# mpetri/ans-large-alphabet

Hardware: AMD Instinct MI355X
Metric: encode+decode Mints/s (uint32), bit-exact vs CPU reference per block (higher is better)
Workload: dtype u32 symbols; ANS state carried as an exact f64 (integers below 2^53) in the encoder, u64 in the decoder; 1 GPU; ANSfold-1 on 268435456 uint32 per GPU, zipf20s1.2, blocks of 16384 ints, restart every 1024; codec=ANSfold-1, ints_per_gpu=268435456, distribution=zipf20s1.2, block_ints=16384, ckpt_interval=1024, seed=1234, multi_gpu=single GPU

## Files before the change

### ans_large_alphabet_amd/csrc/ansx.hip

```cpp
#include "../../include/ansx.h"

#include <hip/hip_runtime.h>
#include <dlfcn.h>
#include <rccl/rccl.h>

#include <algorithm>
#include <array>
#include <cmath>
#include <cstdio>
#include <cstdlib>
#include <cstring>
#include <deque>
#include <map>
#include <set>
#include <string>
#include <vector>

#include "ansx_kernels.h"
#include "ansx_rfold.h"
#include "ansx_model.h"
#include "ansx_fastmodel.h"
#include "ansx_gen.h"
#include "ansx_pa.h"
#include "ansx_intsparse.h"
// ... 22 lines not shown
    hipStream_t stream = nullptr;
    int last_hip = 0;
    bool profile = false;
    std::vector<ProfRec> recs;
    std::map<std::string, std::pair<double, u64>> acc;
    std::vector<std::string> order;
    DevBuf pre_work;
    DevBuf hist, hterm, sortF, sortSym, attS, prevS, attMeta, blk, table, tab32, scratch, misc, mapped, mostfreq,
        stage_in, stage_out, dec_s2s, dec_cum, dec_info, plain, rf_tmp, log2lut, pa_alpha, pa_info, pairs, lg2i, sizes, nearlist, force;
    u32* h_pin = nullptr;
    std::map<u64, u32> ns_hint;
    std::map<u64, u32> rf_hint;
    std::map<std::array<u64, 4>, ansx_container_header> hdr_cache;
    std::deque<std::array<u64, 4>> hdr_order;
    std::map<u32, DevBuf> geo;
    DevBuf geo_big;
    u32 geo_big_cap = 0;
    int last_gather_ranks = 0;
    std::set<u64> wide_hint;
    std::map<u64, u32> t_hint;
    const u32* cur_force = nullptr;
    const u32* cur_src = nullptr;
    bool used_pc = false;
    bool used_fast = false;
    u32 cur_nt = 0;
    u32 cur_rf_slots = 0;
    u32 cur_pa_distinct = 0;
    std::set<u64> int_sparse_hint;
    bool cur_int_sparse = false;
    u32 sp_retries = 0;
    bool sp_full_lds = false;
    ansx_encode_stats last = {};
    struct {
        bool table16_fixup = false;
        bool encode_gtab16 = false;
        bool parse_generic = false;
        bool parse_win = false;
        bool parse_fast = false;
        bool decode_table = false;
        bool no_stream_lds = false;
        int decode_mode = 0;
        u32 parse_stage_words = 0;
        bool model_fused = false;
        bool model_sync = false;
        bool use_pc = false;
        u32 pc_b_pairs = 2;
        u32 test_sp_bits = 0;
        bool fin_one_wave = false;
        bool no_big_geo = false;
        bool no_pc_auto = false;
        bool encode_mode2 = false;
        bool force_pc = false;
        bool no_pc = false;
        int decode_small_ring = 0;
        int decode_pair = 0;
        u32 pair_lds_limit = 0;
        u32 wide_at = 16;
        bool wide_restart = false;
        u32 ns_hint = 0;
        u32 t_hint = 0;
        bool no_fast_model = false;
        double near_band = ANSX_NEAR_BAND;
        bool near_flip = false;
        u32 cand_chains = 0;
        double fast_guard = ANSX_FAST_GUARD;
    } dbg;
};

namespace {

#define HIPCHK(ctx, call)                                                                        \
    do {                                                                                         \
        hipError_t _e = (call);                                                                  \
        if (_e != hipSuccess) {                                                                  \
            (ctx)->last_hip = (int)_e;                                                           \
            return ANSX_ERR_HIP;                                                                 \
        }                                                                                        \
    } while (0)

int ensure(ansx_ctx* c, DevBuf& b, size_t bytes)
{
    if (bytes <= b.cap) return ANSX_OK;
    if (b.p) {
        hipError_t e = hipFree(b.p);
        b.p = nullptr;
        b.cap = 0;
        if (e != hipSuccess) {
            c->last_hip = (int)e;
            return ANSX_ERR_HIP;
        }
    }
    size_t want = bytes + (bytes >> 3) + 4096;
    hipError_t e = hipMalloc(&b.p, want);
    if (e != hipSuccess) {
        c->last_hip = (int)e;
        return ANSX_ERR_HIP;
    }
    b.cap = want;
    return ANSX_OK;
}

void prof_begin(ansx_ctx* c, const char* name, hipStream_t s)
{
    if (!c->profile) return;
    ProfRec r;
    r.name = name;
// ... 153 lines not shown
        LAUNCH(c, "k_rfg_insert", k_rfg_insert, grid, 256, 0, s, d_in, g, slots, keys, counts, bstat);
        if ((size_t)T * 8 > 48 * 1024)
            HIPCHK(c, hipFuncSetAttribute((const void*)k_rfg_select,
                          hipFuncAttributeMaxDynamicSharedMemorySize, (int)((size_t)T * 8)));
        LAUNCH(c, "k_rfg_select", k_rfg_select, g.nblocks, 256, (size_t)T * 8, s, g, slots, (const u32*)keys,
            counts, (const u32*)bstat, mostfreq, blk, gflags);
        LAUNCH(c, "k_rfg_map", k_rfg_map, grid, 256, 0, s, d_in, g, slots, (const u32*)keys, (const u32*)counts,
            (const ansx_blk*)blk, mapped);
        return ANSX_OK;
    }
    if (T <= 4096) {
        const size_t sel_bytes = 8 * (size_t)(T < 512 ? 512 : T);
        if (opt_slots != 0 && opt_slots < ANSX_RF_SLOTS) {
            const size_t lds = 6 * (size_t)opt_slots + sel_bytes;
            HIPCHK(c, hipFuncSetAttribute((const void*)k_rfold_remap_hash2,
                          hipFuncAttributeMaxDynamicSharedMemorySize, (int)lds));
#ifdef ANSX_STAMPS_RF
            { static unsigned long long z[3] = { 0, 0, 0 }; (void)hipMemcpyToSymbol(HIP_SYMBOL(g_stamps), z, 24, 4101 * 8); }
            hipEvent_t e0, e1; (void)hipEventCreate(&e0); (void)hipEventCreate(&e1); (void)hipEventRecord(e0, s);
#endif
            LAUNCH(c, "k_rfold_remap", k_rfold_remap_hash2, g.nblocks, 1024, lds, s, d_in, g, opt_slots, mapped,
                mostfreq, blk, gflags);
#ifdef ANSX_STAMPS_RF
            {
                (void)hipEventRecord(e1, s); (void)hipStreamSynchronize(s);
                float ms = 0; (void)hipEventElapsedTime(&ms, e0, e1);
                unsigned long long z[3]; (void)hipMemcpyFromSymbol(z, HIP_SYMBOL(g_stamps), 24, 4101 * 8);
                fprintf(stderr, "[stamps] k_rfold_remap_hash2: events %.3f ms; workgroup lifetimes: max %llu ticks, mean %.0f ticks, %llu above 40 us\n", ms, z[0], (double)z[1] / g.nblocks, z[2]);
            }
#endif
            return ANSX_OK;
        }
        const size_t lds = 6 * (size_t)ANSX_RF_SLOTS + sel_bytes;
        HIPCHK(c, hipFuncSetAttribute((const void*)k_rfold_remap_hash,
                      hipFuncAttributeMaxDynamicSharedMemorySize, (int)lds));
        LAUNCH(c, "k_rfold_remap", k_rfold_remap_hash, g.nblocks, 1024, lds, s, d_in, g, (u32)ANSX_RF_SLOTS, mapped,
            mostfreq, blk, gflags);
        return ANSX_OK;
    }
    u32 N2 = 2;
    while (N2 < g.block_ints) N2 <<= 1;
    size_t lds = 6 * (size_t)N2 + 8 * (size_t)T + 16;
    if (lds > 48 * 1024)
        HIPCHK(c, hipFuncSetAttribute((const void*)k_rfold_remap,
                      hipFuncAttributeMaxDynamicSharedMemorySize, (int)lds));
    LAUNCH(c, "k_rfold_remap_sort", k_rfold_remap, g.nblocks, 256, lds, s, d_in, g, N2, mapped, mostfreq,
        blk, gflags);
    return ANSX_OK;
}

constexpr int ANSX_RETRY_GENERAL = -1;
constexpr int ANSX_RETRY_WIDE = -2;

template <bool POW2, int S>
static int launch_pc(ansx_ctx* c, const ansx_geo& g, u32 NSP, const u32* src, u32 ns_entries, u32 rowwords, u32 pairs, u32 wgs,
    size_t lds, ansx_blk* blk, u64 scr_stride, u64* ck_state, u32* ck_off, u32* enc_sizes, unsigned long long* enc_gsums, hipStream_t s)
{
    HIPCHK(c, hipFuncSetAttribute((const void*)k_encode_pc<POW2, S>, hipFuncAttributeMaxDynamicSharedMemorySize, (int)lds));
    LAUNCH(c, "k_encode", (k_encode_pc<POW2, S>), wgs, 128 * pairs, lds, s, src, g, NSP, (const u32*)c->tab32.p, ns_entries, rowwords, blk,
        (u8*)c->scratch.p, scr_stride, ck_state, ck_off, enc_sizes, enc_gsums);
    return ANSX_OK;
}
static int launch_f64_encoder(ansx_ctx* c, const ansx_geo& g, u32 NSP, const u32* src, u32 ns_entries, ansx_blk* blk, u64 scr_stride,
    u64* ck_state, u32* ck_off, u32* enc_sizes, unsigned long long* enc_gsums, u32 NB, hipStream_t s)
{
    c->used_pc = false;
    const u32 lds_stride = ns_entries | 1u;
    const size_t enc_lds = (size_t)16 * lds_stride * 4;
    const bool mode1 = enc_lds <= 40 * 1024 && !c->dbg.encode_mode2;
    const bool pow2 = map_is_pow2(g.map);
    int rc;
    u32 first = 0;
    const u32 rowwords = ((ns_entries + 2u) / 2u) | 1u;
    const u32 full_blocks = (u32)(g.n / g.block_ints);
    const u32 enc_waves_all = (NB + 15) / 16;
    auto pc_lds = [&](u32 pairs, u32 S) { return (size_t)pairs * 16 * rowwords * 4 + (size_t)pairs * (2 * S * 1024 + (S == 8 ? 16 * 144 : 0)); };
    u32 pairs = 0, S = 0;
    const bool pc_geo = !c->dbg.no_pc && g.block_ints % 128u == 0 && g.block_ints <= (1u << 22) && (u64)scr_stride * 16 < 0x40000000ull;
    if (pc_geo && (!c->dbg.no_pc_auto || c->dbg.use_pc || c->dbg.force_pc) && mode1 && pc_lds(4, 8) <= 160 * 1024
        && (((NB + 63) / 64) * 2 >= (u32)c->num_cus || c->dbg.force_pc))
        pairs = 4, S = 8;
    else if (pc_geo && !mode1 && pc_lds(2, 4) <= 160 * 1024 && (full_blocks >= 32 || c->dbg.force_pc) && !c->dbg.no_pc_auto)
        pairs = c->dbg.pc_b_pairs, S = 4;
    else if (pc_geo && mode1 && enc_waves_all <= 2u * (u32)c->num_cus && (full_blocks >= 16 || c->dbg.force_pc) && !c->dbg.no_pc_auto)
        pairs = 1, S = 8;
    if (pairs && (g.ckpt == 0 || g.ckpt % (4u * S) == 0)) {
        const u32 wgs = (NB + 16 * pairs - 1) / (16 * pairs);
        const size_t lds = pc_lds(pairs, S);
        if (pow2) rc = S == 8 ? launch_pc<true, 8>(c, g, NSP, src, ns_entries, rowwords, pairs, wgs, lds, blk, scr_stride, ck_state, ck_off, enc_sizes, enc_gsums, s)
                              : launch_pc<true, 4>(c, g, NSP, src, ns_entries, rowwords, pairs, wgs, lds, blk, scr_stride, ck_state, ck_off, enc_sizes, enc_gsums, s);
        else rc = S == 8 ? launch_pc<false, 8>(c, g, NSP, src, ns_entries, rowwords, pairs, wgs, lds, blk, scr_stride, ck_state, ck_off, enc_sizes, enc_gsums, s)
                         : launch_pc<false, 4>(c, g, NSP, src, ns_entries, rowwords, pairs, wgs, lds, blk, scr_stride, ck_state, ck_off, enc_sizes, enc_gsums, s);
        if (rc) return rc;
        first = wgs * 16 * pairs;
        c->used_pc = true;
        if (first >= NB) return ANSX_OK;
    }
    const u32 enc_waves = (NB - first + 15) / 16;
    u32 wpw = (enc_waves + c->num_cus - 1) / c->num_cus;
    wpw = wpw < 1 ? 1 : (wpw > 4 ? 4 : wpw);
    const size_t enc_grid = (enc_waves + wpw - 1) / wpw;
    if (mode1) {
        if (wpw * enc_lds > 48 * 1024) {
            HIPCHK(c, hipFuncSetAttribute((const void*)k_encode<1, true>, hipFuncAttributeMaxDynamicSharedMemorySize, (int)(wpw * enc_lds)));
            HIPCHK(c, hipFuncSetAttribute((const void*)k_encode<1, false>, hipFuncAttributeMaxDynamicSharedMemorySize, (int)(wpw * enc_lds)));
        }
        if (pow2)
            LAUNCH(c, first ? "k_encode_rest" : "k_encode", (k_encode<1, true>), enc_grid, 64 * wpw, wpw * enc_lds, s, src, g, NSP,
                (const ansx_enc_entry*)nullptr, (const u32*)c->tab32.p, lds_stride, blk, (u8*)c->scratch.p,
                (u64)scr_stride, ck_state, ck_off, enc_sizes, enc_gsums, first);
        else
            LAUNCH(c, first ? "k_encode_rest" : "k_encode", (k_encode<1, false>), enc_grid, 64 * wpw, wpw * enc_lds, s, src, g, NSP,
                (const ansx_enc_entry*)nullptr, (const u32*)c->tab32.p, lds_stride, blk, (u8*)c->scratch.p,
                (u64)scr_stride, ck_state, ck_off, enc_sizes, enc_gsums, first);
        return ANSX_OK;
    }
    const size_t lds2 = (size_t)wpw * 16 * ANSX_ENC_HOT * 4;
    if (lds2 > 48 * 1024)
        HIPCHK(c, hipFuncSetAttribute((const void*)k_encode<2>, hipFuncAttributeMaxDynamicSharedMemorySize, (int)lds2));
    LAUNCH(c, first ? "k_encode_rest" : "k_encode_gtab", (k_encode<2>), enc_grid, 64 * wpw, lds2, s, src, g, NSP,
        (const ansx_enc_entry*)nullptr, (const u32*)c->tab32.p, (u32)ANSX_ENC_HOT, blk, (u8*)c->scratch.p,
        (u64)scr_stride, ck_state, ck_off, enc_sizes, enc_gsums, first);
    return ANSX_OK;
}

int encode_general(ansx_ctx* c, const Plan& P, const u32* d_in, u8* d_out, size_t cap,
    size_t* out_bytes, hipStream_t s, u32* seen_ns, u32 ns_cap)
{
    const bool optimistic = ns_cap != 0;
    const ansx_geo& g = P.g;
    const u32 NB = g.nblocks, NSP = P.NSP, f = g.f;
    const size_t scr_stride = rup(block_bound(g.kind, f, g.block_ints, g.pa != 0) + 16, 256);
    if (!P.plain && cap < P.lay.payload_off) return ANSX_ERR_CAPACITY;
    int rc;
    if ((rc = ensure(c, c->hist, (size_t)NB * NSP * 4))) return rc;
    if ((rc = ensure(c, c->sortF, (size_t)NB * NSP * 4))) return rc;
    if ((rc = ensure(c, c->sortSym, (size_t)NB * NSP * 2))) return rc;
    const size_t fbytes = g.kind == ANSX_INT ? 4 : 2;
    if ((rc = ensure(c, c->attS, (size_t)NB * ANSX_ATTEMPTS * NSP * fbytes))) return rc;
    if ((rc = ensure(c, c->prevS, (size_t)NB * NSP * fbytes))) return rc;
    if ((rc = ensure(c, c->attMeta, (size_t)NB * ANSX_ATTEMPTS * 16))) return rc;
    if (!c->log2lut.p) {
// ... 1141 lines not shown
            for (int w = 0; w < 256; w++) {
                if (!h[w * 16] || !h[w * 16 + last]) continue;
                nn++;
                for (int i = 1; i <= last; i++) acc[i] += (double)(h[w * 16 + i] - h[w * 16 + i - 1]);
            }
            fprintf(stderr, "[stamps] %d workgroups, 100 MHz ticks per phase:", nn);
            for (int i = 1; i <= 10; i++) fprintf(stderr, " %d:%.0f", i, nn ? acc[i] / nn : 0.0);
#ifdef ANSX_STAMPS_RF
            { double a9 = 0, a10 = 0, a2 = 0; int m = 0; for (int w = 0; w < 256; w++) if (h[w*16+9] && h[w*16+10] && h[w*16+1]) { a9 += (double)(h[w*16+9]-h[w*16+1]); a10 += (double)(h[w*16+10]-h[w*16+9]); a2 += (double)(h[w*16+2]-h[w*16+10]); m++; }
              if (m) fprintf(stderr, "  [insert split: clear %.0f count %.0f merge %.0f]", a9/m, a10/m, a2/m); }
#endif
            fprintf(stderr, "\n");
#ifdef ANSX_STAMPS_RF
            {
                unsigned long long t0 = ~0ull, t1 = 0;
                for (int w = 0; w < 256; w++) if (h[w * 16] && h[w * 16 + 8]) { t0 = std::min(t0, h[w * 16]); t1 = std::max(t1, h[w * 16 + 8]); }
                fprintf(stderr, "[stamps] rfold: first start .. last end = %llu ticks\n", t1 - t0);
                for (int w = 0; w < 256; w += 8)
                    fprintf(stderr, "[stamps]  wg %5d start %7llu dur %5llu xcc %llx\n", w * 61 + 7, h[w * 16] - t0, h[w * 16 + 8] - h[w * 16], h[w * 16 + 9]);
            }
#endif
            double cc = 0, cl = 0, ct = 0;
            int n2 = 0;
            for (int w = 0; w < 256; w++)
                if (h[w * 16 + 14]) cc += (double)h[w * 16 + 12], cl += (double)h[w * 16 + 13], ct += (double)h[w * 16 + 14], n2++;
            if (n2) fprintf(stderr, "[stamps] k_candidates (%d waves): commit %.0f loop %.0f total %.0f ticks\n", n2, cc / n2, cl / n2, ct / n2);
        }
    }
#endif
    return ANSX_OK;
}

int ansx_debug_set(ansx_ctx* c, const char* name, const char* value)
{
    if (!c || !name) return ANSX_ERR_ARG;
    const bool on = value != nullptr && value[0] != 0 && strcmp(value, "0") != 0;
    if (!strcmp(name, "ANSX_TEST_TABLE16_FIXUP")) c->dbg.table16_fixup = on;
    else if (!strcmp(name, "ANSX_ENCODE_GTAB16")) c->dbg.encode_gtab16 = on;
    else if (!strcmp(name, "ANSX_PARSE_GENERIC")) c->dbg.parse_generic = on;
    else if (!strcmp(name, "ANSX_PARSE_WIN")) c->dbg.parse_win = on;
    else if (!strcmp(name, "ANSX_PARSE_FAST")) c->dbg.parse_fast = on;
    else if (!strcmp(name, "ANSX_DECODE_TABLE")) c->dbg.decode_table = on;
    else if (!strcmp(name, "ANSX_NO_STREAM_LDS")) c->dbg.no_stream_lds = on;
    else if (!strcmp(name, "ANSX_MODEL_FUSED")) c->dbg.model_fused = on;
    else if (!strcmp(name, "ANSX_MODEL_SYNC")) c->dbg.model_sync = on;
    else if (!strcmp(name, "ANSX_DECODE_MODE"))
        c->dbg.decode_mode = !value ? 0 : !strcmp(value, "ring") ? 1 : !strcmp(value, "staged") ? 2 : 0;
    else if (!strcmp(name, "ANSX_PARSE_STAGE_WORDS")) c->dbg.parse_stage_words = value ? (u32)strtoul(value, nullptr, 10) : 0u;
    else if (!strcmp(name, "ANSX_NS_HINT")) c->dbg.ns_hint = value ? (u32)strtoul(value, nullptr, 10) : 0u;
    else if (!strcmp(name, "ANSX_T_HINT")) c->dbg.t_hint = value ? (u32)strtoul(value, nullptr, 10) : 0u;
    else if (!strcmp(name, "ANSX_NO_FAST_MODEL")) c->dbg.no_fast_model = on;
    else if (!strcmp(name, "ANSX_WIDE_RESTART")) c->dbg.wide_restart = on;
    else if (!strcmp(name, "ANSX_NO_PC")) c->dbg.no_pc = on;
    else if (!strcmp(name, "ANSX_FORCE_PC")) c->dbg.force_pc = on;
    else if (!strcmp(name, "ANSX_USE_PC")) c->dbg.use_pc = on;
    else if (!strcmp(name, "ANSX_NO_PC_AUTO")) c->dbg.no_pc_auto = on;
    else if (!strcmp(name, "ANSX_NO_BIG_GEO")) c->dbg.no_big_geo = on;
    else if (!strcmp(name, "ANSX_FIN_ONE_WAVE")) c->dbg.fin_one_wave = on;
    else if (!strcmp(name, "ANSX_TEST_SP_BITS")) c->dbg.test_sp_bits = value ? (u32)atoi(value) : 0u;
    else if (!strcmp(name, "ANSX_PC_B_PAIRS")) c->dbg.pc_b_pairs = (value && value[0] == '1') ? 1u : 2u;
    else if (!strcmp(name, "ANSX_ENCODE_MODE2")) c->dbg.encode_mode2 = on;
    else if (!strcmp(name, "ANSX_DECODE_SMALL_RING"))
        c->dbg.decode_small_ring = !value ? 0 : !strcmp(value, "never") ? 1 : !strcmp(value, "always") ? 2 : 0;
    else if (!strcmp(name, "ANSX_DECODE_PAIR"))
        c->dbg.decode_pair = !value ? 0 : !strcmp(value, "never") ? 1 : !strcmp(value, "always") ? 2 : 0;
    else if (!strcmp(name, "ANSX_DECODE_PAIR_LDS")) c->dbg.pair_lds_limit = (value && value[0]) ? (u32)strtoul(value, nullptr, 10) : 0u;
    else if (!strcmp(name, "ANSX_FORGET_HINTS")) {
        c->ns_hint.clear();
        c->rf_hint.clear();
        c->t_hint.clear();
        c->wide_hint.clear();
        c->hdr_cache.clear();
        c->hdr_order.clear();
    }
    else if (!strcmp(name, "ANSX_TEST_WIDE_AT")) {
        const u32 v = (value && value[0]) ? (u32)strtoul(value, nullptr, 10) : 16u;
        if (v > 16) return ANSX_ERR_ARG;
        c->dbg.wide_at = v;
    }
    else if (!strcmp(name, "ANSX_NEAR_BAND")) c->dbg.near_band = (value && value[0]) ? strtod(value, nullptr) : ANSX_NEAR_BAND;
    else if (!strcmp(name, "ANSX_TEST_NEAR_FLIP")) c->dbg.near_flip = on;
    else if (!strcmp(name, "ANSX_CAND_CHAINS")) {
        const u32 v = value ? (u32)strtoul(value, nullptr, 10) : 0u;
        if (v > 2) return ANSX_ERR_ARG;
        c->dbg.cand_chains = v;
    } else if (!strcmp(name, "ANSX_FAST_GUARD")) c->dbg.fast_guard = (value && value[0]) ? strtod(value, nullptr) : ANSX_FAST_GUARD;
    else return ANSX_ERR_ARG;
    return ANSX_OK;
}

void ansx_destroy(ansx_ctx* c)
{
    if (!c) return;
    (void)hipSetDevice(c->device);
    (void)hipStreamSynchronize(c->stream);
    DevBuf* bufs[] = { &c->pre_work, &c->hist, &c->hterm, &c->sortF, &c->sortSym, &c->attS, &c->prevS, &c->attMeta, &c->blk,
        &c->table, &c->tab32, &c->scratch, &c->misc, &c->mapped, &c->mostfreq, &c->stage_in, &c->stage_out,
        &c->dec_s2s, &c->dec_cum, &c->dec_info, &c->plain, &c->rf_tmp, &c->log2lut, &c->pa_alpha, &c->pa_info, &c->pairs, &c->lg2i, &c->sizes, &c->nearlist, &c->force, &c->geo_big };
    for (DevBuf* b : bufs)
        if (b->p) (void)hipFree(b->p);
    for (auto& kv : c->geo)
        if (kv.second.p) (void)hipFree(kv.second.p);
    for (auto& r : c->recs) {
        (void)hipEventDestroy(r.e0);
        (void)hipEventDestroy(r.e1);
    }
// ... 418 lines not shown
```

### ans_large_alphabet_amd/csrc/ansx_kernels.h

```cpp
#pragma once

#include <type_traits>

#include "ansx_dev.h"

#ifdef ANSX_STAMPS
__device__ unsigned long long g_stamps[16 * 256 + 16];
#define STAMP(i) do { if (threadIdx.x == 0 && blockIdx.x % 61 == 7 && blockIdx.x / 61 < 256) g_stamps[(blockIdx.x / 61) * 16 + (i)] = wall_clock64(); } while (0)
#else
#define STAMP(i) do { } while (0)
#endif
#ifdef ANSX_STAMPS_RF
#define STAMP_RF(i) STAMP(i)
#else
#define STAMP_RF(i) do { } while (0)
#endif

struct ansx_blk {
    u32 n;
    u32 max_sym;
    u32 sigma;
    u32 m0_log2;
    double H;
    double thr;
// ... 1724 lines not shown
                } else {
#pragma unroll
                    for (int j = 0; j < ANSX_ENC_U; j++) e0[j] = e1[j];
                    if (sb + 1 < ANSX_ENC_XB / ANSX_ENC_U) {
#pragma unroll
                        for (int j = 0; j < ANSX_ENC_U; j++)
                            e1[j] = tab.getp(f, xa[(sb + 1) * ANSX_ENC_U + j], Md, 8 * ql);
                    }
                }
                const u32 sbtop = top - sb * ANSX_ENC_U;
                if (ck_per_batch) {
#pragma unroll
                    for (int j = 0; j < ANSX_ENC_U; j++)
                        tab.step_nb(L, xa[sb * ANSX_ENC_U + j], e0[j], qc, ql, logM, rsrc, out);
                    record(sbtop - ANSX_ENC_U);
                } else {
#pragma unroll
                    for (int j = 0; j < ANSX_ENC_U; j++) {
                        tab.step_nb(L, xa[sb * ANSX_ENC_U + j], e0[j], qc, ql, logM, rsrc, out);
                        record(sbtop - 1 - j);
                    }
                }
            }
            gi = top - ANSX_ENC_XB;
            asm volatile("s_waitcnt vmcnt(40)" ::: "memory");
#pragma unroll
            for (int j = 0; j < ANSX_ENC_XB; j += 8)
                asm volatile(""
                             : "+v"(xb[j]), "+v"(xb[j + 1]), "+v"(xb[j + 2]), "+v"(xb[j + 3]), "+v"(xb[j + 4]),
                             "+v"(xb[j + 5]), "+v"(xb[j + 6]), "+v"(xb[j + 7]));
#pragma unroll
            for (int j = 0; j < ANSX_ENC_XB; j++) xa[j] = xb[j];
            if constexpr (MODE == 2) {
                if (gi) {
#pragma unroll
                    for (int j = 0; j < ANSX_ENC_U; j++) raw1[j] = tab.fetchp(f, xa[j], raw1l[j]);
                }
            }
        }
        }
        L.p -= pbias;
        pbias = 0;
    }
    st_u64_unaligned(out + L.p + 8 * ql, tab.state(L) - Lb);
    if (ql == 0) publish_size(B, b, L.p + 32);
}

#define ANSX_PC_S 8
__device__ __forceinline__ void quad_transpose4(u32 (&v)[4], u32 ql);
__device__ __forceinline__ void pc_store_short_hi(u32 v, ansx_u32x4 rs, u32 voff)
{
    asm volatile("buffer_store_short_d16_hi %0, %1, %2, 0 offen" : : "v"(v), "v"(voff), "s"(rs) : "memory");
}
template <bool POW2, int S>
__global__ __launch_bounds__(512) void k_encode_pc(const u32* __restrict__ in, ansx_geo g, u32 NSP,
    const u32* __restrict__ tab32, u32 ns_cap, u32 rowwords, ansx_blk* __restrict__ blk, u8* __restrict__ scratch,
    u64 scr_stride, u64* __restrict__ ckpt_state, u32* __restrict__ ckpt_off, u32* __restrict__ sizes,
    unsigned long long* __restrict__ gsums)
{
    static_assert(S == 4 || S == 8, "the input ring is 32 steps deep: 4 or 8 batches per super-batch");
    extern __shared__ u32 lds_pc[];
    typedef __attribute__((address_space(3))) u16 lds_u16;
    typedef __attribute__((address_space(3))) ansx_u32x4 lds_x4;
    const u32 lane = threadIdx.x & 63u, wv = threadIdx.x >> 6;
    const u32 pairs = blockDim.x >> 7;
    const bool producer = wv >= pairs;
    const u32 pair = producer ? wv - pairs : wv;
    const u32 wb0 = (u32)__builtin_amdgcn_readfirstlane((int)((blockIdx.x * pairs + pair) * 16));
    u32* const ptab = lds_pc + pair * 16 * rowwords;
    constexpr u32 HANDW = 2 * S * 64 * 4 + (S == 8 ? 16 * 36 : 0);
    u32* const hand = lds_pc + pairs * 16 * rowwords + pair * HANDW;
    {
        const u32 r0 = producer ? 8u : 0u;
        const u32 lim = ns_cap < NSP ? ns_cap : NSP;
        for (u32 j = 0; j < 8; j++) {
            if (wb0 + r0 + j >= g.nblocks) break;
            const u32* row0 = tab32 + (u64)(wb0 + r0 + j) * NSP;
            lds_u16* c0 = (lds_u16*)(ptab + (r0 + j) * rowwords);
            for (u32 e0 = 0; e0 < lim; e0 += 640) {
                u32 v0[10];
#pragma unroll
                for (int i = 0; i < 10; i++) {
                    const u32 e = e0 + lane + 64 * i;
                    v0[i] = e < lim ? row0[e] : 0u;
                }
#pragma unroll
                for (int i = 0; i < 10; i++) {
                    const u32 e = e0 + lane + 64 * i;
                    if (e < lim) c0[e + 1] = (u16)((v0[i] >> 16) + (v0[i] & 0xFFFFu));
                }
            }
            if (lane == 0) c0[0] = 0;
        }
    }
    __syncthreads();
    const u32 b = wb0 + (lane >> 2), ql = lane & 3u;
    const u32 G = g.block_ints >> 2;
    const bool irr = (u64)(blockIdx.x + 1) * 16u * pairs * g.block_ints > g.n;
    const u32 Gtot = G + (irr ? (u32)ANSX_ENC_XB : 0u);
    const u32 NBATCH = Gtot / (u32)S;
    const bool exists = b < g.nblocks;
    const u32 nbk = exists ? geo_block_n(g, b) : 0u;
    const u32 Gp = nbk >> 2, rt = nbk & 3u;
    if (producer) {
        const ansx_map f = g.map;
        const u64 iba = (u64)(uintptr_t)(in + (u64)wb0 * g.block_ints);
        const u64 ifirst = (u64)wb0 * g.block_ints;
        const u64 irem = ifirst < g.n ? g.n - ifirst : 0;
        const u32 inrec = (u32)((irem < 16ull * g.block_ints ? irem : 16ull * g.block_ints) * 4);
        const ansx_u32x4 irs = ansx_u32x4{ (u32)__builtin_amdgcn_readfirstlane((u32)iba),
            (u32)__builtin_amdgcn_readfirstlane((u32)(iba >> 32) & 0xFFFFu), (u32)__builtin_amdgcn_readfirstlane(inrec), 0x00020000u };
        const u32 tbase = (u32)(uintptr_t)(__attribute__((address_space(3))) const u32*)ptab + 4 * (lane >> 2) * rowwords;
        const u32 hbase = (u32)(uintptr_t)(__attribute__((address_space(3))) const u32*)hand + 16 * lane;
        const u32 lgm = (exists && irr) ? blk[b].logM : 8u;
        ansx_u32x4 neutral = ansx_u32x4{ 0u, 0u, 0u, 0u };
        if (irr) {
            const u32 Mn = lgm <= 15 ? (1u << lgm) : 65535u;
            const double Md_ = (double)Mn;
            const double r0 = __builtin_amdgcn_rcp(Md_);
            const double rc = __builtin_fma(__builtin_fma(-Md_, r0, 1.0 - 1.8189894035458565e-12), r0, r0);
            neutral = ansx_u32x4{ f64_lo(rc) & ~3u, f64_hi(rc), Mn, 0u };
        }
        const u32* const tailp = in + (u64)(exists ? b : 0) * g.block_ints + 3u * Gp;
        auto fix_x = [&](u32 x, u32 gi) -> u32 {
            const bool real = gi < Gp, tail = !real && ql == 0 && gi < Gp + rt;
            u32 tv = 0;
            if (__builtin_amdgcn_ballot_w64(tail) != 0) tv = tail ? tailp[gi] : 0u;
            return real ? x : tv;
        };
        auto fix_h = [&](const ansx_u32x4& h, u32 gi) -> ansx_u32x4 {
            const bool live = gi < Gp || (ql == 0 && gi < Gp + rt);
            return live ? h : neutral;
        };
        const u32 c32f = 8u + (u32)__builtin_clz(f.t1);
        auto entry = [&](u32 x, u32 k, u32 sh, u32 cur, u32 nxt) {
            const u32 F = (nxt - cur) & 0xFFFFu;
            const double Fd = (double)F;
            const double r0 = __builtin_amdgcn_rcp(Fd);
            const double rc = __builtin_fma(__builtin_fma(-Fd, r0, 1.0 - 1.8189894035458565e-12), r0, r0);
            ansx_u32x4 h;
            h.x = (f64_lo(rc) & ~3u) | k;
            h.y = f64_hi(rc);
            h.z = F | (cur << 16);
            const u32 xs = x >> (sh & 8u);
            h.w = (x & 0xFFu) | (xs << 16);
            return h;
        };
        auto fold_of = [&](u32 x, u32& k, u32& sh) {
            if constexpr (POW2) {
                const u32 d = __builtin_elementwise_sub_sat(c32f, ffbh_u32(x));
                k = d >> 3;
                sh = d & 0x18u;
            } else {
                k = map_nbytes(f, x);
                sh = k << 3;
            }
            return tbase + 2 * (__umul24(k, f.D) + (x >> sh));
        };
        u32 pb = 0;
        const u32 rtl = ql == 0 ? rt : 0u;
        auto emit = [&](u32 (&x)[S], u32 gtop, u32 hb) {
            bool act = true;
            if (irr) {
                const bool real = gtop <= Gp, neut = gtop - (u32)S >= Gp + rtl;
                if (__builtin_amdgcn_ballot_w64(!real && !neut) != 0) {
                    u32 kk[S], shh[S], cur[S], nxt[S];
#pragma unroll
                    for (int i = 0; i < S; i++) x[i] = fix_x(x[i], gtop - 1u - (u32)i);
#pragma unroll
                    for (int i = 0; i < S; i++) {
                        const u32 la = fold_of(x[i], kk[i], shh[i]);
                        cur[i] = *(lds_u16*)(size_t)la;
                        nxt[i] = *(lds_u16*)(size_t)(la + 2);
                    }
#pragma unroll
                    for (int i = 0; i < S; i++) *(lds_x4*)(size_t)(hb + i * 1024) = fix_h(entry(x[i], kk[i], shh[i], cur[i], nxt[i]), gtop - 1u - (u32)i);
                    return;
                }
                if (pb < 2 && neut) {
#pragma unroll
                    for (int i = 0; i < S; i++) *(lds_x4*)(size_t)(hb + i * 1024) = neutral;
                }
                act = real;
            }
            if (act) {
                u32 kk[S], shh[S], cur[S], nxt[S];
#pragma unroll
                for (int i = 0; i < S; i++) {
                    const u32 la = fold_of(x[i], kk[i], shh[i]);
                    cur[i] = *(lds_u16*)(size_t)la;
                    nxt[i] = *(lds_u16*)(size_t)(la + 2);
                }
#pragma unroll
                for (int i = 0; i < S; i++) *(lds_x4*)(size_t)(hb + i * 1024) = entry(x[i], kk[i], shh[i], cur[i], nxt[i]);
            }
        };
        if constexpr (S == 8) {
            u32* const strip = hand + 2 * S * 64 * 4 + 0;
            const u32 sbase = (u32)(uintptr_t)(__attribute__((address_space(3))) const u32*)strip + (lane >> 2) * 144;
            const u32 vq = (lane >> 2) * g.block_ints * 4 + 32 * ql;
            ansx_u32x4 w[4][2];
            auto request = [&](u32 batch, ansx_u32x4 (&d)[2]) {
                const u32 off = vq + 16u * (Gtot - 8u * batch - 8u);
                asm volatile("buffer_load_dwordx4 %0, %1, %2, 0 offen" : "=v"(d[0]) : "v"(off), "s"(irs) : "memory");
                asm volatile("buffer_load_dwordx4 %0, %1, %2, 0 offen offset:16" : "=v"(d[1]) : "v"(off), "s"(irs) : "memory");
            };
            request(0, w[0]);
            request(1, w[1]);
            request(2, w[2]);
            for (u32 sb = 0; sb < Gtot / ANSX_ENC_XB; sb++) {
#pragma unroll
                for (int t = 0; t < 4; t++) {
                    request(pb + 3, w[(t + 3) % 4]);
                    asm volatile("s_waitcnt vmcnt(6)" : "+v"(w[t][0]), "+v"(w[t][1]) : : "memory");
                    *(lds_x4*)(size_t)(sbase + 32 * ql) = w[t][0];
                    *(lds_x4*)(size_t)(sbase + 32 * ql + 16) = w[t][1];
                    u32 xx[8];
#pragma unroll
                    for (int i = 0; i < 8; i++) xx[i] = *(__attribute__((address_space(3))) const u32*)(size_t)(sbase + 16 * (7 - i) + 4 * (3 - ql));
                    emit(xx, Gtot - 8u * pb, hbase + (pb & 1u) * (S * 1024));
                    pb++;
                    __syncthreads();
                }
            }
            asm volatile("s_waitcnt vmcnt(0)" : "+v"(w[0][0]), "+v"(w[0][1]), "+v"(w[1][0]), "+v"(w[1][1]), "+v"(w[2][0]), "+v"(w[2][1]), "+v"(w[3][0]), "+v"(w[3][1]) : : "memory");
            return;
        }
        if constexpr (S == 4) {
        const u32 vq4 = (lane >> 2) * g.block_ints * 4 + 16u * (3u - ql);
        ansx_u32x4 wq[8];
        auto request4 = [&](u32 batch, ansx_u32x4& d) {
            const u32 off = vq4 + 16u * (Gtot - 4u * batch - 4u);
            asm volatile("buffer_load_dwordx4 %0, %1, %2, 0 offen" : "=v"(d) : "v"(off), "s"(irs) : "memory");
        };
#pragma unroll
        for (int j = 0; j < 7; j++) request4((u32)j, wq[j]);
        for (u32 sb = 0; sb < Gtot / ANSX_ENC_XB; sb++) {
#pragma unroll
            for (int t = 0; t < 8; t++) {
                request4(pb + 7, wq[(t + 7) % 8]);
                asm volatile("s_waitcnt vmcnt(7)" : "+v"(wq[t]) : : "memory");
                u32 xs_[4] = { wq[t].w, wq[t].z, wq[t].y, wq[t].x };
                quad_transpose4(xs_, ql);
                emit(xs_, Gtot - 4u * pb, hbase + (pb & 1u) * (S * 1024));
                pb++;
                __syncthreads();
            }
        }
        asm volatile("s_waitcnt vmcnt(0)" : "+v"(wq[0]), "+v"(wq[1]), "+v"(wq[2]), "+v"(wq[3]), "+v"(wq[4]), "+v"(wq[5]), "+v"(wq[6]), "+v"(wq[7]) : : "memory");
        }
        return;
    }
    ansx_blk* B = &blk[exists ? b : 0];
    const bool skip = !exists || B->status || !B->resolved || B->pa_sigma == 1;
    const u32 logM = exists ? B->logM : 8u;
    const u64 Lb = (u64)16 << logM;
    const double Md = (double)(1u << logM);
    const __amdgpu_buffer_rsrc_t rsrc = __builtin_amdgcn_make_buffer_rsrc(
        scratch + (u64)wb0 * scr_stride, 0, (int)(16 * scr_stride), 0x00020000);
    const u64 sba = (u64)(uintptr_t)(scratch + (u64)wb0 * scr_stride);
    const ansx_u32x4 srs = ansx_u32x4{ (u32)__builtin_amdgcn_readfirstlane((u32)sba), (u32)__builtin_amdgcn_readfirstlane((u32)(sba >> 32) & 0xFFFFu),
        (u32)__builtin_amdgcn_readfirstlane((u32)(16 * scr_stride)), 0x00020000u };
    const u32 obase = (u32)((lane >> 2) * scr_stride);
    u8* out = scratch + (u64)b * scr_stride;
    const u32 cg = g.ckpt >> 2;
    u32 ck_seg = (cg && Gp && !skip) ? (Gp - 1) / cg : 0;
    u32 ck_g = ck_seg * cg;
    const u32 pbias = obase;
    double sd = (double)Lb;
    u32 pcur = skip ? 0x40000000u : B->prelude_bytes + obase;
    auto record = [&](u32 gidx) {
        if (ck_seg && gidx == ck_g) {
            const u64 idx = (u64)b * g.nckf + (ck_seg - 1);
            const u64 stv = f64_to_u64_exact(sd);
            if (g.ckw) {
                ckpt_state[idx * 4 + ql] = stv;
                if (ql == 0) ckpt_off[idx] = pcur - pbias;
            } else {
                u8* rec = (u8*)ckpt_state + idx * ANSX_CK_RECORD;
                const u64 pst = ((u64)quad_perm<ANSX_QP(1, 0, 3, 2)>((u32)(stv >> 32)) << 32) | quad_perm<ANSX_QP(1, 0, 3, 2)>((u32)stv);
                if ((ql & 1u) == 0) {
                    u8* pp = rec + 13u * (ql >> 1);
                    st_u64_unaligned(pp, (stv & ((1ull << ANSX_CK_STATE_BITS) - 1ull)) | (pst << ANSX_CK_STATE_BITS));
                    st_u32_unaligned(pp + 8, (u32)(pst >> 12));
                    pp[12] = (u8)(pst >> 44);
                }
                if (ql == 0) {
                    const u32 cur = pcur - pbias;
                    st_u16_unaligned(rec + 26, (u16)cur);
                    rec[28] = (u8)(cur >> 16);
                }
            }
            ck_seg--;
            ck_g -= cg;
        }
    };
    const u32 hbase = (u32)(uintptr_t)(__attribute__((address_space(3))) const u32*)hand + 16 * lane;
    const u32 four_pos = 4u << (8 * ql), lomask = (1u << (8 * ql)) - 1u, ql8 = 8 * ql;
    u32 gi = Gtot;
    const u32 gstart = Gp + (ql == 0 ? rt : 0u);
    const double sd_first = sd;
    const bool creeps = irr && logM == 16;
    auto steps = [&](auto RESET, u32 hb) {
        ansx_u32x4 h[S];
#pragma unroll
        for (int i = 0; i < S; i++) h[i] = *(lds_x4*)(size_t)(hb + i * 1024);
#pragma unroll
        for (int i = 0; i < S; i++) {
            const u32 k = h[i].x & 3u;
            const double rcp = __builtin_bit_cast(double, ((u64)h[i].y << 32) | h[i].x);
            const double Fd = (double)(h[i].z & 0xFFFFu);
            const double based = (double)(h[i].z >> 16);
            const u32 thr_hi = f64_hi(Fd) + (36u << 20);
            const double MF = Md - Fd, omF = 1.0 - Fd;
            const u32 off1 = (h[i].x << 31) + ANSX_BUF_OOB;
            const u32 off2 = (k - 2u) & 0x80000001u;
            if constexpr (decltype(RESET)::value) sd = gi - (u32)i == gstart ? sd_first : sd;
            const bool rn = f64_hi(sd) >= thr_hi;
            const u32 w = f64_lo(sd + 4503599627370496.0);
            int ex = rn ? -32 : 0;
            asm("" : "+v"(ex));
            const double s0 = __builtin_trunc(__builtin_ldexp(sd, ex));
            const double q = __builtin_trunc(s0 * rcp);
            const double base2 = __builtin_fma(q, MF, s0 + based);
            const double one_short = __builtin_fmin(__builtin_fmax(__builtin_fma(-q, Fd, s0 + omF), 0.0), 1.0);
            sd = __builtin_fma(one_short, MF, base2);
            const u32 v = (k << ql8) + (rn ? four_pos : 0u);
            const u32 s1 = quad_add_dpp<0xB1>(v);
            const u32 Sq = quad_add_dpp<0x4E>(s1);
            const u32 a = __builtin_amdgcn_sad_u8(Sq & lomask, 0u, pcur);
            pcur = __builtin_amdgcn_sad_u8(Sq, 0u, pcur);
#ifndef ANSX_PC_ABL_NOSTORE
            __builtin_amdgcn_raw_buffer_store_b8((u8)h[i].w, rsrc, a + off1, 0, 0);
            pc_store_short_hi(h[i].w, srs, a + off2);
            __builtin_amdgcn_raw_buffer_store_b32(w, rsrc, rn ? a + k : ANSX_BUF_OOB, 0, 0);
#else
            asm volatile("" :: "v"(a + off1), "v"(a + off2), "v"(rn ? a + k : ANSX_BUF_OOB), "v"(w));
#endif
        }
    };
    for (u32 cb = 0; cb < NBATCH; cb++) {
        __syncthreads();
        const u32 hb = hbase + (cb & 1u) * (S * 1024);
        if (irr && __builtin_amdgcn_ballot_w64(creeps && gstart <= gi && gstart + (u32)S > gi) != 0) steps(std::true_type{}, hb);
        else steps(std::false_type{}, hb);
        gi -= (u32)S;
        record(gi);
    }
    if (!exists) return;
    if (skip) {
        if (ql == 0) {
            const u32 sz = (B->pa_sigma == 1 && !B->status) ? B->pre_bytes : 0u;
            B->stream_bytes = sz;
            sizes[b] = sz;
            if (sz) atomicAdd(&gsums[b >> 6], (unsigned long long)sz);
        }
        return;
    }
    const u32 pfin = pcur - pbias;
    st_u64_unaligned(out + pfin + 8 * ql, f64_to_u64_exact(sd) - Lb);
    if (ql == 0) {
        const u32 sz = pfin + 32;
        B->stream_bytes = sz;
        sizes[b] = sz;
        atomicAdd(&gsums[b >> 6], (unsigned long long)sz);
    }
}

__global__ __launch_bounds__(1024) void k_scan_sizes(ansx_geo g, const ansx_blk* __restrict__ blk,
    u64* __restrict__ block_off, u64* __restrict__ result, u64 payload_off, u64 capacity,
    u32* __restrict__ gflags)
{
    __shared__ u64 part[20];
    const u32 tid = threadIdx.x, lane = tid & 63, wave = tid >> 6;
    const u32 NB = g.nblocks;
    const u32 per = ((NB + 15) / 16 + 63) & ~63u;
    const u32 lo = wave * per < NB ? wave * per : NB, hi = (lo + per) < NB ? (lo + per) : NB;
    u64 sum = 0;
    for (u32 i = lo + lane; i < hi; i += 64) sum += blk[i].stream_bytes;
    sum = wave_sum(sum);
    u64 total;
    u64 run = block_excl_scan<u64>(lane == 63 ? sum : 0ull, part, tid, 1024, &total);
    run = wave_last(run);
    if (tid == 0) {
        block_off[NB] = total;
        result[0] = total;
        if (payload_off + total > capacity) atomicOr(&gflags[ANSX_G_ERR], 1u << 2 );
    }
    for (u32 i0 = lo; i0 < hi; i0 += 64) {
        const u32 i = i0 + lane;
        const u64 v = i < hi ? (u64)blk[i].stream_bytes : 0ull;
        const u64 incl = wave_incl_scan(v);
        if (i < hi) block_off[i] = run + incl - v;
        run += wave_last(incl);
    }
}

__global__ __launch_bounds__(256) void k_compact(ansx_geo g, const ansx_blk* __restrict__ blk,
// ... 1741 lines not shown
```

Before: 140,100 Mints/s.

## Shrink producer-consumer handoff to 8 bytes with LDS reciprocal table

```diff
diff --git a/ans_large_alphabet_amd/csrc/ansx.hip b/ans_large_alphabet_amd/csrc/ansx.hip
--- a/ans_large_alphabet_amd/csrc/ansx.hip
+++ b/ans_large_alphabet_amd/csrc/ansx.hip
@@ -98,6 +98,7 @@
         bool encode_mode2 = false;
         bool force_pc = false;
         bool no_pc = false;
+        bool no_pc_rt = false;
         int decode_small_ring = 0;
         int decode_pair = 0;
         u32 pair_lds_limit = 0;
@@ -357,12 +358,12 @@
 constexpr int ANSX_RETRY_GENERAL = -1;
 constexpr int ANSX_RETRY_WIDE = -2;
 
-template <bool POW2, int S>
+template <bool POW2, int S, bool RT = false>
 static int launch_pc(ansx_ctx* c, const ansx_geo& g, u32 NSP, const u32* src, u32 ns_entries, u32 rowwords, u32 pairs, u32 wgs,
     size_t lds, ansx_blk* blk, u64 scr_stride, u64* ck_state, u32* ck_off, u32* enc_sizes, unsigned long long* enc_gsums, hipStream_t s)
 {
-    HIPCHK(c, hipFuncSetAttribute((const void*)k_encode_pc<POW2, S>, hipFuncAttributeMaxDynamicSharedMemorySize, (int)lds));
-    LAUNCH(c, "k_encode", (k_encode_pc<POW2, S>), wgs, 128 * pairs, lds, s, src, g, NSP, (const u32*)c->tab32.p, ns_entries, rowwords, blk,
+    HIPCHK(c, hipFuncSetAttribute((const void*)k_encode_pc<POW2, S, RT>, hipFuncAttributeMaxDynamicSharedMemorySize, (int)lds));
+    LAUNCH(c, "k_encode", (k_encode_pc<POW2, S, RT>), wgs, 128 * pairs, lds, s, src, g, NSP, (const u32*)c->tab32.p, ns_entries, rowwords, blk,
         (u8*)c->scratch.p, scr_stride, ck_state, ck_off, enc_sizes, enc_gsums);
     return ANSX_OK;
 }
@@ -380,6 +381,7 @@
     const u32 full_blocks = (u32)(g.n / g.block_ints);
     const u32 enc_waves_all = (NB + 15) / 16;
     auto pc_lds = [&](u32 pairs, u32 S) { return (size_t)pairs * 16 * rowwords * 4 + (size_t)pairs * (2 * S * 1024 + (S == 8 ? 16 * 144 : 0)); };
+    auto pc_lds_rt = [&](u32 pairs) { return (size_t)pairs * 16 * rowwords * 4 + (size_t)pairs * (2 * 8 * 512 + 16 * 144) + (size_t)ANSX_PC_FTAB * 8 + 32; };
     u32 pairs = 0, S = 0;
     const bool pc_geo = !c->dbg.no_pc && g.block_ints % 128u == 0 && g.block_ints <= (1u << 22) && (u64)scr_stride * 16 < 0x40000000ull;
     if (pc_geo && (!c->dbg.no_pc_auto || c->dbg.use_pc || c->dbg.force_pc) && mode1 && pc_lds(4, 8) <= 160 * 1024
@@ -391,8 +393,11 @@
         pairs = 1, S = 8;
     if (pairs && (g.ckpt == 0 || g.ckpt % (4u * S) == 0)) {
         const u32 wgs = (NB + 16 * pairs - 1) / (16 * pairs);
-        const size_t lds = pc_lds(pairs, S);
-        if (pow2) rc = S == 8 ? launch_pc<true, 8>(c, g, NSP, src, ns_entries, rowwords, pairs, wgs, lds, blk, scr_stride, ck_state, ck_off, enc_sizes, enc_gsums, s)
+        const bool rt = pairs == 4 && S == 8 && !c->dbg.no_pc_rt && pc_lds_rt(4) <= 160 * 1024;
+        const size_t lds = rt ? pc_lds_rt(pairs) : pc_lds(pairs, S);
+        if (rt) rc = pow2 ? launch_pc<true, 8, true>(c, g, NSP, src, ns_entries, rowwords, pairs, wgs, lds, blk, scr_stride, ck_state, ck_off, enc_sizes, enc_gsums, s)
+                          : launch_pc<false, 8, true>(c, g, NSP, src, ns_entries, rowwords, pairs, wgs, lds, blk, scr_stride, ck_state, ck_off, enc_sizes, enc_gsums, s);
+        else if (pow2) rc = S == 8 ? launch_pc<true, 8>(c, g, NSP, src, ns_entries, rowwords, pairs, wgs, lds, blk, scr_stride, ck_state, ck_off, enc_sizes, enc_gsums, s)
                               : launch_pc<true, 4>(c, g, NSP, src, ns_entries, rowwords, pairs, wgs, lds, blk, scr_stride, ck_state, ck_off, enc_sizes, enc_gsums, s);
         else rc = S == 8 ? launch_pc<false, 8>(c, g, NSP, src, ns_entries, rowwords, pairs, wgs, lds, blk, scr_stride, ck_state, ck_off, enc_sizes, enc_gsums, s)
                          : launch_pc<false, 4>(c, g, NSP, src, ns_entries, rowwords, pairs, wgs, lds, blk, scr_stride, ck_state, ck_off, enc_sizes, enc_gsums, s);
@@ -1640,6 +1645,7 @@
     else if (!strcmp(name, "ANSX_NO_FAST_MODEL")) c->dbg.no_fast_model = on;
     else if (!strcmp(name, "ANSX_WIDE_RESTART")) c->dbg.wide_restart = on;
     else if (!strcmp(name, "ANSX_NO_PC")) c->dbg.no_pc = on;
+    else if (!strcmp(name, "ANSX_NO_PC_RT")) c->dbg.no_pc_rt = on;
     else if (!strcmp(name, "ANSX_FORCE_PC")) c->dbg.force_pc = on;
     else if (!strcmp(name, "ANSX_USE_PC")) c->dbg.use_pc = on;
     else if (!strcmp(name, "ANSX_NO_PC_AUTO")) c->dbg.no_pc_auto = on;
diff --git a/ans_large_alphabet_amd/csrc/ansx_kernels.h b/ans_large_alphabet_amd/csrc/ansx_kernels.h
--- a/ans_large_alphabet_amd/csrc/ansx_kernels.h
+++ b/ans_large_alphabet_amd/csrc/ansx_kernels.h
@@ -1800,24 +1800,45 @@
 {
     asm volatile("buffer_store_short_d16_hi %0, %1, %2, 0 offen" : : "v"(v), "v"(voff), "s"(rs) : "memory");
 }
-template <bool POW2, int S>
+__device__ __forceinline__ double pc_rcp_under(double Fd)
+{
+    const double r0 = __builtin_amdgcn_rcp(Fd);
+    const double rc = __builtin_fma(__builtin_fma(-Fd, r0, 1.0 - 1.8189894035458565e-12), r0, r0);
+    return __builtin_bit_cast(double, __builtin_bit_cast(u64, rc) & ~3ull);
+}
+#define ANSX_PC_FTAB 4096u
+typedef u32 ansx_u32x2 __attribute__((ext_vector_type(2)));
+template <bool POW2, int S, bool RT>
 __global__ __launch_bounds__(512) void k_encode_pc(const u32* __restrict__ in, ansx_geo g, u32 NSP,
     const u32* __restrict__ tab32, u32 ns_cap, u32 rowwords, ansx_blk* __restrict__ blk, u8* __restrict__ scratch,
     u64 scr_stride, u64* __restrict__ ckpt_state, u32* __restrict__ ckpt_off, u32* __restrict__ sizes,
     unsigned long long* __restrict__ gsums)
 {
     static_assert(S == 4 || S == 8, "the input ring is 32 steps deep: 4 or 8 batches per super-batch");
+    static_assert(!RT || S == 8, "the RT form is the four-pair shape's");
     extern __shared__ u32 lds_pc[];
     typedef __attribute__((address_space(3))) u16 lds_u16;
     typedef __attribute__((address_space(3))) ansx_u32x4 lds_x4;
+    typedef __attribute__((address_space(3))) ansx_u32x2 lds_x2;
+    typedef __attribute__((address_space(3))) u32 lds_u32;
+    typedef __attribute__((address_space(3))) double lds_f64;
     const u32 lane = threadIdx.x & 63u, wv = threadIdx.x >> 6;
     const u32 pairs = blockDim.x >> 7;
     const bool producer = wv >= pairs;
     const u32 pair = producer ? wv - pairs : wv;
     const u32 wb0 = (u32)__builtin_amdgcn_readfirstlane((int)((blockIdx.x * pairs + pair) * 16));
-    u32* const ptab = lds_pc + pair * 16 * rowwords;
-    constexpr u32 HANDW = 2 * S * 64 * 4 + (S == 8 ? 16 * 36 : 0);
-    u32* const hand = lds_pc + pairs * 16 * rowwords + pair * HANDW;
+    u32* const ftab = lds_pc;
+    u32* const bflag = ftab + 2 * ANSX_PC_FTAB + 2 * pair;
+    u32* const lds0 = lds_pc + (RT ? 2 * ANSX_PC_FTAB + 8 : 0u);
+    u32* const ptab = lds0 + pair * 16 * rowwords;
+    constexpr u32 EW = RT ? 2 : 4;
+    constexpr u32 EB = 64 * 4 * EW;
+    constexpr u32 HANDW = 2 * S * 64 * EW + (S == 8 ? 16 * 36 : 0);
+    u32* const hand = lds0 + pairs * 16 * rowwords + pair * HANDW;
+    if constexpr (RT) {
+        for (u32 F = threadIdx.x; F < ANSX_PC_FTAB; F += blockDim.x)
+            ((lds_f64*)(__attribute__((address_space(3))) u32*)ftab)[F] = pc_rcp_under((double)F);
+    }
     {
         const u32 r0 = producer ? 8u : 0u;
         const u32 lim = ns_cap < NSP ? ns_cap : NSP;
@@ -1859,15 +1880,16 @@
         const ansx_u32x4 irs = ansx_u32x4{ (u32)__builtin_amdgcn_readfirstlane((u32)iba),
             (u32)__builtin_amdgcn_readfirstlane((u32)(iba >> 32) & 0xFFFFu), (u32)__builtin_amdgcn_readfirstlane(inrec), 0x00020000u };
         const u32 tbase = (u32)(uintptr_t)(__attribute__((address_space(3))) const u32*)ptab + 4 * (lane >> 2) * rowwords;
-        const u32 hbase = (u32)(uintptr_t)(__attribute__((address_space(3))) const u32*)hand + 16 * lane;
+        const u32 hbase = (u32)(uintptr_t)(__attribute__((address_space(3))) const u32*)hand + 4 * EW * lane;
+        const u32 fbase = (u32)(uintptr_t)(__attribute__((address_space(3))) const u32*)bflag;
         const u32 lgm = (exists && irr) ? blk[b].logM : 8u;
         ansx_u32x4 neutral = ansx_u32x4{ 0u, 0u, 0u, 0u };
+        ansx_u32x2 neutral2 = ansx_u32x2{ 0u, 0u };
         if (irr) {
             const u32 Mn = lgm <= 15 ? (1u << lgm) : 65535u;
-            const double Md_ = (double)Mn;
-            const double r0 = __builtin_amdgcn_rcp(Md_);
-            const double rc = __builtin_fma(__builtin_fma(-Md_, r0, 1.0 - 1.8189894035458565e-12), r0, r0);
-            neutral = ansx_u32x4{ f64_lo(rc) & ~3u, f64_hi(rc), Mn, 0u };
+            const double rc = pc_rcp_under((double)Mn);
+            neutral = ansx_u32x4{ f64_lo(rc), f64_hi(rc), Mn, 0u };
+            neutral2 = ansx_u32x2{ Mn, 0u };
         }
         const u32* const tailp = in + (u64)(exists ? b : 0) * g.block_ints + 3u * Gp;
         auto fix_x = [&](u32 x, u32 gi) -> u32 {
@@ -1876,23 +1898,42 @@
             if (__builtin_amdgcn_ballot_w64(tail) != 0) tv = tail ? tailp[gi] : 0u;
             return real ? x : tv;
         };
-        auto fix_h = [&](const ansx_u32x4& h, u32 gi) -> ansx_u32x4 {
+        auto fix_h = [&](const auto& h, u32 gi) {
             const bool live = gi < Gp || (ql == 0 && gi < Gp + rt);
-            return live ? h : neutral;
+            if constexpr (RT) return live ? h : neutral2;
+            else return live ? h : neutral;
         };
         const u32 c32f = 8u + (u32)__builtin_clz(f.t1);
         auto entry = [&](u32 x, u32 k, u32 sh, u32 cur, u32 nxt) {
             const u32 F = (nxt - cur) & 0xFFFFu;
-            const double Fd = (double)F;
-            const double r0 = __builtin_amdgcn_rcp(Fd);
-            const double rc = __builtin_fma(__builtin_fma(-Fd, r0, 1.0 - 1.8189894035458565e-12), r0, r0);
-            ansx_u32x4 h;
-            h.x = (f64_lo(rc) & ~3u) | k;
-            h.y = f64_hi(rc);
-            h.z = F | (cur << 16);
             const u32 xs = x >> (sh & 8u);
-            h.w = (x & 0xFFu) | (xs << 16);
-            return h;
+            if constexpr (RT) {
+                return ansx_u32x2{ F | (cur << 16), (x & 0xFFu) | (k << 8) | (xs << 16) };
+            } else {
+                const double rc = pc_rcp_under((double)F);
+                ansx_u32x4 h;
+                h.x = f64_lo(rc) | k;
+                h.y = f64_hi(rc);
+                h.z = F | (cur << 16);
+                h.w = (x & 0xFFu) | (xs << 16);
+                return h;
+            }
+        };
+        u32 fo = 0;
+        auto put = [&](u32 hb, int i, const auto& h) {
+            if constexpr (RT) {
+                fo |= h.x & 0xFFFFu;
+                *(lds_x2*)(size_t)(hb + i * EB) = h;
+            } else {
+                *(lds_x4*)(size_t)(hb + i * EB) = h;
+            }
+        };
+        auto put_flag = [&](u32 par) {
+            if constexpr (RT) {
+                const bool big = irr || __builtin_amdgcn_ballot_w64(fo >= ANSX_PC_FTAB) != 0;
+                *(lds_u32*)(size_t)(fbase + 4 * par) = big ? 1u : 0u;
+                fo = 0;
+            }
         };
         auto fold_of = [&](u32 x, u32& k, u32& sh) {
             if constexpr (POW2) {
@@ -1922,12 +1963,15 @@
                         nxt[i] = *(lds_u16*)(size_t)(la + 2);
                     }
 #pragma unroll
-                    for (int i = 0; i < S; i++) *(lds_x4*)(size_t)(hb + i * 1024) = fix_h(entry(x[i], kk[i], shh[i], cur[i], nxt[i]), gtop - 1u - (u32)i);
+                    for (int i = 0; i < S; i++) put(hb, i, fix_h(entry(x[i], kk[i], shh[i], cur[i], nxt[i]), gtop - 1u - (u32)i));
                     return;
                 }
                 if (pb < 2 && neut) {
 #pragma unroll
-                    for (int i = 0; i < S; i++) *(lds_x4*)(size_t)(hb + i * 1024) = neutral;
+                    for (int i = 0; i < S; i++) {
+                        if constexpr (RT) put(hb, i, neutral2);
+                        else put(hb, i, neutral);
+                    }
                 }
                 act = real;
             }
@@ -1940,11 +1984,11 @@
                     nxt[i] = *(lds_u16*)(size_t)(la + 2);
                 }
 #pragma unroll
-                for (int i = 0; i < S; i++) *(lds_x4*)(size_t)(hb + i * 1024) = entry(x[i], kk[i], shh[i], cur[i], nxt[i]);
+                for (int i = 0; i < S; i++) put(hb, i, entry(x[i], kk[i], shh[i], cur[i], nxt[i]));
             }
         };
         if constexpr (S == 8) {
-            u32* const strip = hand + 2 * S * 64 * 4 + 0;
+            u32* const strip = hand + 2 * S * 64 * EW;
             const u32 sbase = (u32)(uintptr_t)(__attribute__((address_space(3))) const u32*)strip + (lane >> 2) * 144;
             const u32 vq = (lane >> 2) * g.block_ints * 4 + 32 * ql;
             ansx_u32x4 w[4][2];
@@ -1966,7 +2010,8 @@
                     u32 xx[8];
 #pragma unroll
                     for (int i = 0; i < 8; i++) xx[i] = *(__attribute__((address_space(3))) const u32*)(size_t)(sbase + 16 * (7 - i) + 4 * (3 - ql));
-                    emit(xx, Gtot - 8u * pb, hbase + (pb & 1u) * (S * 1024));
+                    emit(xx, Gtot - 8u * pb, hbase + (pb & 1u) * (S * EB));
+                    put_flag(pb & 1u);
                     pb++;
                     __syncthreads();
                 }
@@ -1990,7 +2035,7 @@
                 asm volatile("s_waitcnt vmcnt(7)" : "+v"(wq[t]) : : "memory");
                 u32 xs_[4] = { wq[t].w, wq[t].z, wq[t].y, wq[t].x };
                 quad_transpose4(xs_, ql);
-                emit(xs_, Gtot - 4u * pb, hbase + (pb & 1u) * (S * 1024));
+                emit(xs_, Gtot - 4u * pb, hbase + (pb & 1u) * (S * EB));
                 pb++;
                 __syncthreads();
             }
@@ -2043,7 +2088,7 @@
             ck_g -= cg;
         }
     };
-    const u32 hbase = (u32)(uintptr_t)(__attribute__((address_space(3))) const u32*)hand + 16 * lane;
+    const u32 hbase = (u32)(uintptr_t)(__attribute__((address_space(3))) const u32*)hand + 4 * EW * lane;
     const u32 four_pos = 4u << (8 * ql), lomask = (1u << (8 * ql)) - 1u, ql8 = 8 * ql;
     u32 gi = Gtot;
     const u32 gstart = Gp + (ql == 0 ? rt : 0u);
@@ -2052,7 +2097,7 @@
     auto steps = [&](auto RESET, u32 hb) {
         ansx_u32x4 h[S];
 #pragma unroll
-        for (int i = 0; i < S; i++) h[i] = *(lds_x4*)(size_t)(hb + i * 1024);
+        for (int i = 0; i < S; i++) h[i] = *(lds_x4*)(size_t)(hb + i * EB);
 #pragma unroll
         for (int i = 0; i < S; i++) {
             const u32 k = h[i].x & 3u;
@@ -2087,11 +2132,67 @@
 #endif
         }
     };
+    auto steps_rt = [&](auto RESET, auto TAB, u32 hb) {
+        ansx_u32x2 h[S];
+        double rct[S];
+#pragma unroll
+        for (int i = 0; i < S; i++) h[i] = *(lds_x2*)(size_t)(hb + i * EB);
+        if constexpr (decltype(TAB)::value) {
+#pragma unroll
+            for (int i = 0; i < S; i++) {
+                u32 ad;
+                asm("v_lshlrev_b32 %0, 3, %1" : "=v"(ad) : "v"(h[i].x & 0xFFFFu));
+                rct[i] = *(lds_f64*)(size_t)ad;
+            }
+        }
+#pragma unroll
+        for (int i = 0; i < S; i++) {
+            const u32 k = (h[i].y >> 8) & 3u;
+            const double Fd = (double)(h[i].x & 0xFFFFu);
+            const double rcp = decltype(TAB)::value ? rct[i] : pc_rcp_under(Fd);
+            const double based = (double)(h[i].x >> 16);
+            const u32 thr_hi = f64_hi(Fd) + (36u << 20);
+            const double MF = Md - Fd, omF = 1.0 - Fd;
+            const u32 off1 = (k << 31) + ANSX_BUF_OOB;
+            const u32 off2 = (k - 2u) & 0x80000001u;
+            if constexpr (decltype(RESET)::value) sd = gi - (u32)i == gstart ? sd_first : sd;
+            const bool rn = f64_hi(sd) >= thr_hi;
+            const u32 w = f64_lo(sd + 4503599627370496.0);
+            int ex = rn ? -32 : 0;
+            asm("" : "+v"(ex));
+            const double s0 = __builtin_trunc(__builtin_ldexp(sd, ex));
+            const double q = __builtin_trunc(s0 * rcp);
+            const double base2 = __builtin_fma(q, MF, s0 + based);
+            const double one_short = __builtin_fmin(__builtin_fmax(__builtin_fma(-q, Fd, s0 + omF), 0.0), 1.0);
+            sd = __builtin_fma(one_short, MF, base2);
+            const u32 v = (k << ql8) + (rn ? four_pos : 0u);
+            const u32 s1 = quad_add_dpp<0xB1>(v);
+            const u32 Sq = quad_add_dpp<0x4E>(s1);
+            const u32 a = __builtin_amdgcn_sad_u8(Sq & lomask, 0u, pcur);
+            pcur = __builtin_amdgcn_sad_u8(Sq, 0u, pcur);
+#ifndef ANSX_PC_ABL_NOSTORE
+            __builtin_amdgcn_raw_buffer_store_b8((u8)h[i].y, rsrc, a + off1, 0, 0);
+            pc_store_short_hi(h[i].y, srs, a + off2);
+            __builtin_amdgcn_raw_buffer_store_b32(w, rsrc, rn ? a + k : ANSX_BUF_OOB, 0, 0);
+#else
+            asm volatile("" :: "v"(a + off1), "v"(a + off2), "v"(rn ? a + k : ANSX_BUF_OOB), "v"(w));
+#endif
+        }
+    };
+    const u32 fbase = (u32)(uintptr_t)(__attribute__((address_space(3))) const u32*)bflag;
     for (u32 cb = 0; cb < NBATCH; cb++) {
         __syncthreads();
-        const u32 hb = hbase + (cb & 1u) * (S * 1024);
-        if (irr && __builtin_amdgcn_ballot_w64(creeps && gstart <= gi && gstart + (u32)S > gi) != 0) steps(std::true_type{}, hb);
-        else steps(std::false_type{}, hb);
+        const u32 hb = hbase + (cb & 1u) * (S * EB);
+        const bool reset = irr && __builtin_amdgcn_ballot_w64(creeps && gstart <= gi && gstart + (u32)S > gi) != 0;
+        if constexpr (RT) {
+            const u32 big = (u32)__builtin_amdgcn_readfirstlane((int)*(lds_u32*)(size_t)(fbase + 4 * (cb & 1u)));
+            if (reset) steps_rt(std::true_type{}, std::false_type{}, hb);
+            else if (big) steps_rt(std::false_type{}, std::false_type{}, hb);
+            else steps_rt(std::false_type{}, std::true_type{}, hb);
+        } else {
+            if (reset) steps(std::true_type{}, hb);
+            else steps(std::false_type{}, hb);
+        }
         gi -= (u32)S;
         record(gi);
     }
```

Result: no change. 139,700 Mints/s, median of 6 (-0.3%).
